# facebookresearch/actionmesh

Measured on AMD Instinct MI355X. Metric: denoise-steps/sec (16f x 4096tok), higher is better.
Workload: dtype bf16; 1 GPU; headline: Stage-I denoise step, B=2 (CFG) x T=16 frames x N=4096 tokens, width 1024 (8 heads x 128), 21 layers all inflated, S=257 ctx tokens, random-init weights, seeded N(0,1) latents/context resident in HBM; parallelism=single GPU

## Files before the change

actionmesh_amd/csrc/am_gemm.hip:

```cpp
#include <stdlib.h>
#include <string.h>

#include "am_common.h"

namespace {

constexpr int BM = 128, BN = 128, BK = 64;
constexpr int LDS_ROW = BK + 8;
constexpr int TILE_ELEMS = BM * LDS_ROW;
constexpr int CS_LD = BN + 4;
constexpr int SMEM_MAIN = 2 * 2 * TILE_ELEMS * (int)sizeof(bf16_t);
constexpr int SMEM_EPI = BM * CS_LD * (int)sizeof(float);
constexpr int SMEM_BYTES = SMEM_MAIN > SMEM_EPI ? SMEM_MAIN : SMEM_EPI;
constexpr int GROUP_M = 8;
constexpr int B2 = 256;

__device__ inline int64_t map_row(int r, int G, int gs, int off) {
  if (G <= 0) return r;
  int g = r / G;
  return (int64_t)g * gs + off + (r - g * G);
}

__global__ __launch_bounds__(256, 2) void gemm_bf16_kernel(am_gemm_args p, int tiles_m, int tiles_n, int m_base) {
  extern __shared__ __attribute__((aligned(16))) unsigned char smem[];
// ... 231 lines not shown
  if (p.residual) {
    const u32x2_t rv = *reinterpret_cast<const u32x2_t*>(p.residual + (int64_t)gmr * p.ldc + gn);
    v[0] += bflo(rv[0]); v[1] += bfhi(rv[0]); v[2] += bflo(rv[1]); v[3] += bfhi(rv[1]);
  }
  *reinterpret_cast<u32x2_t*>(p.C + (int64_t)gmr * p.ldc + gn) = u32x2_t{pack_bf2(v[0], v[1]), pack_bf2(v[2], v[3])};
}

#ifndef AM_GEMM_NT
#define AM_GEMM_NT 1
#endif
struct ResidualPrefetch {
  u32x4_t rv[16];
  bool on;
};
__device__ __forceinline__ bool residual_prefetchable(const am_gemm_args& p, int tid, int m0, int n0) {
  return p.residual != nullptr && p.c_G <= 0 && m0 + B2 <= p.M && n0 + (tid & 31) * 8 < p.N && !(p.act & 0x1800);
}
__device__ __forceinline__ void residual_prefetch(const am_gemm_args& p, int tid, int m0, int n0, ResidualPrefetch& r) {
  r.on = residual_prefetchable(p, tid, m0, n0);
  if (r.on) {
    const int k16 = tid & 31, r16 = tid >> 5;
    const uint32_t lane_off = ((uint32_t)r16 * (uint32_t)p.ldc + (uint32_t)(n0 + k16 * 8)) * 2u;
    const int64_t step = (int64_t)16 * p.ldc;
    const bf16_t* rrow = p.residual + (int64_t)m0 * p.ldc;
#pragma unroll
    for (int pass = 0; pass < 16; ++pass) {
      const u32x4_t* q = reinterpret_cast<const u32x4_t*>(reinterpret_cast<const unsigned char*>(rrow + pass * step) + lane_off);
      r.rv[pass] = AM_GEMM_NT ? __builtin_nontemporal_load(q) : *q;
    }
  }
}

__device__ __forceinline__ void emit_row_part(const u32x4_t& sv, float* part_row, bool writer) {
  float x[8];
#pragma unroll
  for (int e = 0; e < 4; ++e) { x[2 * e] = bflo(sv[e]); x[2 * e + 1] = bfhi(sv[e]); }
  float mean, m2;
  row_part8(x, mean, m2);
#define AM_CHAN_STEP(CTRL, ROWMASK, HALF_N)                                                                                  \
  {                                                                                                                          \
    const float om = __builtin_bit_cast(float, __builtin_amdgcn_update_dpp(__builtin_bit_cast(int, mean), __builtin_bit_cast(int, mean), CTRL, ROWMASK, 0xf, false)); \
    const float oq = __builtin_bit_cast(float, __builtin_amdgcn_update_dpp(__builtin_bit_cast(int, m2), __builtin_bit_cast(int, m2), CTRL, ROWMASK, 0xf, false));     \
    row_part_merge_equal(mean, m2, om, oq, HALF_N);                                                                          \
  }
  AM_CHAN_STEP(0xB1, 0xf, 4.f)
  AM_CHAN_STEP(0x4E, 0xf, 8.f)
  AM_CHAN_STEP(0x141, 0xf, 16.f)
  AM_CHAN_STEP(0x140, 0xf, 32.f)
  AM_CHAN_STEP(0x142, 0xa, 64.f)
#undef AM_CHAN_STEP
  if (writer) *reinterpret_cast<f32x2_t*>(part_row) = f32x2_t{mean, m2};
}

__device__ __forceinline__ void store_staged_tile(const am_gemm_args& p, const unsigned char* stage, int tid, int m0, int n0,
                                                  const ResidualPrefetch* pre = nullptr) {
  {
    const int k16 = tid & 31, r16 = tid >> 5;
    const int gn = n0 + k16 * 8;
    if (gn < p.N) {
      const unsigned char* su = stage + r16 * 512 + ((k16 ^ (r16 >> 1)) << 4);
      const bool odd = r16 & 1;
      auto fetch = [&](int pass) __attribute__((always_inline)) {
        u32x4_t sv = *reinterpret_cast<const u32x4_t*>(su + pass * 8192);
        if (odd) sv = u32x4_t{sv[2], sv[3], sv[0], sv[1]};
        return sv;
      };
      auto add_res = [&](u32x4_t sv, const bf16_t* rp) __attribute__((always_inline)) {
        const u32x4_t rv = *reinterpret_cast<const u32x4_t*>(rp);
#pragma unroll
        for (int e = 0; e < 4; ++e) sv[e] = pack_bf2(bflo(sv[e]) + bflo(rv[e]), bfhi(sv[e]) + bfhi(rv[e]));
// ... 42 lines not shown
        }
      } else {
#pragma unroll 2
        for (int pass = 0; pass < 16; ++pass) {
          const int gmr = m0 + pass * 16 + r16;
          if (gmr < p.M) {
            u32x4_t sv = fetch(pass);
            const int64_t pr = map_row(gmr, p.c_G, p.c_gs, p.c_off);
            if (p.residual) sv = add_res(sv, p.residual + pr * p.ldc + gn);
            *reinterpret_cast<u32x4_t*>(p.C + pr * p.ldc + gn) = sv;
          }
        }
      }
    }
  }
}

__device__ __forceinline__ void store_staged_tile_headpost(const am_gemm_args& p, const am_headpost_args& hp, const unsigned char* stage,
                                                           int tid, int m0, int n0) {
  const int k16 = tid & 31, r16 = tid >> 5;
  const int half = k16 >> 4, sub = k16 & 15;
  const bool abl_noqk = (p.act & 0x800) != 0, abl_nov = (p.act & 0x1000) != 0;
  if (!abl_noqk) {
    const int pi = (n0 >> 7) + half;
    const int head = pi / hp.nparts, part = pi - head * hp.nparts;
    const int kind = (n0 + half * 128 < p.N) ? hp.kinds[part] : 3;
    if (kind == 0 || kind == 1) {
      const float* wt = kind == 0 ? hp.w_q : hp.w_k;
      float wv[8];
#pragma unroll
// ... 310 lines not shown
__device__ __forceinline__ bool gelu_table_has(float x) {
  const uint32_t b = pack_bf2(x, 0.f) & 0x7fffu;
  return b - GT_LO < GT_SPAN;
}

constexpr int HT_BYTES = 128 * BK * 2;
constexpr int PBUF_BYTES = 4 * HT_BYTES;
constexpr int FOLD_OFF = 2 * PBUF_BYTES;
constexpr int SMEM2PP_BYTES = FOLD_OFF + 4096;
constexpr int GT_OFF = SMEM2PP_BYTES;
constexpr int SMEM2PP_GELU_BYTES = GT_OFF + GT_BYTES;

#define PP_BARRIER() do { __builtin_amdgcn_sched_barrier(0); asm volatile("s_barrier" ::: "memory"); __builtin_amdgcn_sched_barrier(0); } while (0)
#define PP_LGKM0() asm volatile("s_waitcnt lgkmcnt(0)" ::: "memory")

template <bool HP>
__global__ __launch_bounds__(512, 2) void gemm256pp_bf16_kernel(am_gemm_args p, int tiles_m, int tiles_n, int m_base, am_headpost_args hp,
                                                                 const uint16_t* gelu_tab) {
  extern __shared__ __attribute__((aligned(16))) unsigned char smem[];

  const int nb = tiles_m * tiles_n;
  const int bid = blockIdx.x;
  {
    const int units = (p.act >> 13) & 7;
    if (units && units < 7 && bid < 256) {
      const unsigned long long t0 = wall_clock64();
      const unsigned long long wait = (unsigned long long)(bid & 7) * units * 150ull;
      while (wall_clock64() - t0 < wait) __builtin_amdgcn_s_sleep(4);
    }
  }
  int lid;
  {
    const int xcd = bid & 7, idx = bid >> 3;
    const int q = nb >> 3, r = nb & 7;
    lid = (xcd < r ? xcd * (q + 1) : r * (q + 1) + (xcd - r) * q) + idx;
  }
  int tm, tn;
  {
    const int group_sz = GROUP_M * tiles_n;
    const int g = lid / group_sz;
    const int first_m = g * GROUP_M;
    const int gm = min(GROUP_M, tiles_m - first_m);
    const int in_g = lid - g * group_sz;
    tm = first_m + in_g % gm;
    tn = in_g / gm;
  }
  const int m0 = m_base + tm * B2, n0 = tn * B2;

  const int tid = threadIdx.x;
  const int lane = tid & 63;
  const int wave = __builtin_amdgcn_readfirstlane(tid >> 6);
  const int wm = wave >> 2, wn = wave & 3;

  const int l15 = lane & 15, l4 = lane >> 4;
  f32x4_t acc[8][4];
  {
    f32x4_t bv[4];
#pragma unroll
    for (int ni = 0; ni < 4; ++ni) {
      bv[ni] = f32x4_t{0.f, 0.f, 0.f, 0.f};
      if (p.bias && !p.ln_stats) bv[ni] = *reinterpret_cast<const f32x4_t*>(p.bias + min(n0 + wn * 64 + ni * 16 + l4 * 4, p.N - 4));
    }
#pragma unroll
    for (int ni = 0; ni < 4; ++ni) asm volatile("" : "+v"(bv[ni]));
#pragma unroll
    for (int ni = 0; ni < 4; ++ni)
#pragma unroll
      for (int mi = 0; mi < 8; ++mi) acc[mi][ni] = bv[ni];
  }
  __builtin_amdgcn_sched_barrier(0);
  if (p.ln_stats) {
    {
      const int dw = wave * 64 + lane;
      const int row = min(m0 + (dw >> 1), p.M - 1);
      __builtin_amdgcn_global_load_lds((gbl_ptr_t)(p.ln_stats + 2 * (int64_t)row + (dw & 1)), (lds_ptr_t)(smem + FOLD_OFF + wave * 256), 4, 0, 0);
    }
    {
      const int idx = (wave & 3) * 64 + lane;
      const int n = min(n0 + idx, p.N - 1);
      const float* src = wave < 4 ? p.ln_colsum + n : (p.bias ? p.bias + n : p.ln_colsum + n);
      __builtin_amdgcn_global_load_lds((gbl_ptr_t)src, (lds_ptr_t)(smem + FOLD_OFF + 2048 + wave * 256), 4, 0, 0);
    }
  }

  if (gelu_tab != nullptr) {
#pragma unroll
    for (int i = 0; i < GT_BYTES / 4 / 512; ++i)
      __builtin_amdgcn_global_load_lds((gbl_ptr_t)(reinterpret_cast<const uint32_t*>(gelu_tab) + i * 512 + wave * 64 + lane),
                                       (lds_ptr_t)(smem + GT_OFF + (i * 512 + wave * 64) * 4), 4, 0, 0);
  }

  uint32_t offA1[4], offA2[4], offW[4];
#pragma unroll
  for (int i = 0; i < 4; ++i) {
    const int half = i >> 1, pc = i & 1;
    const int r = pc * 64 + wave * 8 + (lane >> 3);
    const int c = (lane & 7) ^ ((r >> 1) & 7);
    const int ar = min(m0 + half * 128 + r, p.M - 1);
    const int64_t pr = map_row(ar, p.a_G, p.a_gs, p.a_off);
    offA1[i] = (uint32_t)(pr * (p.lda1 >> 3) + c);
    offA2[i] = (uint32_t)(pr * (p.lda2 >> 3) + c);
    const int wr = min(n0 + half * 128 + r, p.N - 1);
    offW[i] = (uint32_t)((int64_t)wr * (p.ldw >> 3) + c);
  }
  auto stage_a = [&](int half, int kt, int buf_off) __attribute__((always_inline)) {
    const int k0 = kt * BK;
    const bool first = k0 < p.K1;
    const unsigned char* base = reinterpret_cast<const unsigned char*>(first ? p.A1 + k0 : p.A2 + (k0 - p.K1));
#pragma unroll
    for (int pc = 0; pc < 2; ++pc) {
      const uint32_t off = first ? offA1[half * 2 + pc] : offA2[half * 2 + pc];
      __builtin_amdgcn_global_load_lds((gbl_ptr_t)(base + ((uint64_t)off << 4)),
                                       (lds_ptr_t)(smem + buf_off + half * HT_BYTES + (pc * 512 + wave * 64) * 16), 16, 0, 0);
    }
  };
  auto stage_w = [&](int half, int kt, int buf_off) __attribute__((always_inline)) {
    const unsigned char* base = reinterpret_cast<const unsigned char*>(p.W + kt * BK);
#pragma unroll
    for (int pc = 0; pc < 2; ++pc)
      __builtin_amdgcn_global_load_lds((gbl_ptr_t)(base + ((uint64_t)offW[half * 2 + pc] << 4)),
                                       (lds_ptr_t)(smem + buf_off + (2 + half) * HT_BYTES + (pc * 512 + wave * 64) * 16), 16, 0, 0);
  };


  const int fo0 = l15 * 128 + (((0 + l4) ^ (l15 >> 1)) << 4);
  const int fo1 = l15 * 128 + (((4 + l4) ^ (l15 >> 1)) << 4);
  const int a_base = wm * HT_BYTES;
  const int w_base = (2 + (wn >> 1)) * HT_BYTES + (wn & 1) * 64 * 128;

  bf16x8_t af[4][2], wf[4][2];
  auto read_a = [&](int cur, int mh) __attribute__((always_inline)) {
#pragma unroll
    for (int i = 0; i < 4; ++i) {
      const unsigned char* q = smem + cur + a_base + (mh * 4 + i) * 2048;
      af[i][0] = *reinterpret_cast<const bf16x8_t*>(q + fo0);
      af[i][1] = *reinterpret_cast<const bf16x8_t*>(q + fo1);
    }
  };
  auto read_w = [&](int cur, int nh) __attribute__((always_inline)) {
#pragma unroll
    for (int j = 0; j < 2; ++j) {
      const unsigned char* q = smem + cur + w_base + (nh * 2 + j) * 2048;
      wf[nh * 2 + j][0] = *reinterpret_cast<const bf16x8_t*>(q + fo0);
      wf[nh * 2 + j][1] = *reinterpret_cast<const bf16x8_t*>(q + fo1);
    }
  };
#define PP_QUADRANT(MH, NH)                                                                                       \
  do {                                                                                                            \
    __builtin_amdgcn_s_setprio(1);                                                                                \
    _Pragma("unroll") for (int ks = 0; ks < 2; ++ks)                                                              \
      _Pragma("unroll") for (int i = 0; i < 4; ++i)                                                               \
        _Pragma("unroll") for (int j = 0; j < 2; ++j)                                                             \
          acc[(MH) * 4 + i][(NH) * 2 + j] = AM_MFMA_16x16x32(                                                     \
              wf[(NH) * 2 + j][ks], af[i][ks], acc[(MH) * 4 + i][(NH) * 2 + j]);                                  \
    __builtin_amdgcn_s_setprio(0);                                                                                \
  } while (0)

  const int nk = p.K / BK;
  stage_a(0, 0, 0); stage_a(1, 0, 0); stage_w(0, 0, 0); stage_w(1, 0, 0);
  {
    const int t1 = min(1, nk - 1);
    stage_w(0, t1, PBUF_BYTES); stage_w(1, t1, PBUF_BYTES);
  }
  asm volatile("s_waitcnt vmcnt(4)" ::: "memory");
  PP_BARRIER();
  if (wm == 1) PP_BARRIER();

  for (int t = 0; t < nk; ++t) {
    const int cur = (t & 1) * PBUF_BYTES, nxt = PBUF_BYTES - cur;
    const int ta = min(t + 1, nk - 1), tb = min(t + 2, nk - 1);
    read_a(cur, 0); read_w(cur, 0);
    stage_a(0, ta, nxt);
    PP_LGKM0(); PP_BARRIER();
    PP_QUADRANT(0, 0);
    PP_BARRIER();
    read_w(cur, 1);
    stage_a(1, ta, nxt);
    PP_LGKM0(); PP_BARRIER();
    PP_QUADRANT(0, 1);
    PP_BARRIER();
    read_a(cur, 1);
    stage_w(0, tb, cur);
    PP_LGKM0(); PP_BARRIER();
    PP_QUADRANT(1, 1);
    PP_BARRIER();
    stage_w(1, tb, cur);
    asm volatile("s_waitcnt vmcnt(4)" ::: "memory");
    PP_BARRIER();
    PP_QUADRANT(1, 0);
    PP_BARRIER();
  }
  if (wm == 0) PP_BARRIER();
  asm volatile("s_waitcnt vmcnt(0)" ::: "memory");
  PP_BARRIER();

  ResidualPrefetch pre;
  pre.on = false;
  if constexpr (!HP) residual_prefetch(p, tid, m0, n0, pre);
  if (p.ln_stats) {
    f32x4_t cs[4], dv[4];
    const float* fold = reinterpret_cast<const float*>(smem + FOLD_OFF);
#pragma unroll
    for (int ni = 0; ni < 4; ++ni) {
      const int nl = wn * 64 + ni * 16 + l4 * 4;
      cs[ni] = *reinterpret_cast<const f32x4_t*>(fold + 512 + nl);
      dv[ni] = p.bias ? *reinterpret_cast<const f32x4_t*>(fold + 768 + nl) : f32x4_t{0.f, 0.f, 0.f, 0.f};
    }
#pragma unroll
    for (int mi = 0; mi < 8; ++mi) {
      const f32x2_t st = *reinterpret_cast<const f32x2_t*>(fold + 2 * (wm * 128 + mi * 16 + l15));
      const float nm = -st[0] * st[1];
#pragma unroll
      for (int ni = 0; ni < 4; ++ni)
#pragma unroll
        for (int e = 0; e < 4; ++e) acc[mi][ni][e] = fmaf(acc[mi][ni][e], st[1], fmaf(nm, cs[ni][e], dv[ni][e]));
    }
  }
  unsigned char* stage = smem;
  uint32_t gelu_bad = 0;
  auto stage_pass = [&](auto&& convert) __attribute__((always_inline)) {
#pragma unroll
    for (int mi = 0; mi < 8; ++mi)
#pragma unroll
      for (int ni = 0; ni < 4; ++ni) {
        const int ml = wm * 128 + mi * 16 + l15;
        const int nl = wn * 64 + ni * 16 + l4 * 4;
        const u32x2_t w = convert(acc[mi][ni]);
        const int u = (nl >> 2) ^ (ml & 15);
        *reinterpret_cast<u32x2_t*>(stage + ml * 512 + u * 8) = w;
      }
  };
  if ((p.act & 0xff) == 1 && gelu_tab != nullptr) {
    stage_pass([&](const f32x4_t& a) __attribute__((always_inline)) {
      return u32x2_t{gelu_table_pair(pack_bf2(a[0], a[1]), smem + GT_OFF, gelu_bad), gelu_table_pair(pack_bf2(a[2], a[3]), smem + GT_OFF, gelu_bad)};
    });
  } else if ((p.act & 0xff) == 1) {
    stage_pass([&](const f32x4_t& a) __attribute__((always_inline)) {
      float v[4];
#pragma unroll
      for (int e = 0; e < 4; ++e) v[e] = gelu_erf(rbf(a[e]));
      return u32x2_t{pack_bf2(v[0], v[1]), pack_bf2(v[2], v[3])};
    });
  } else {
    stage_pass([&](const f32x4_t& a) __attribute__((always_inline)) { return u32x2_t{pack_bf2(a[0], a[1]), pack_bf2(a[2], a[3])}; });
  }
  if (gelu_bad) {
#pragma unroll
    for (int mi = 0; mi < 8; ++mi)
#pragma unroll
      for (int ni = 0; ni < 4; ++ni) {
        const int ml = wm * 128 + mi * 16 + l15;
        const int nl = wn * 64 + ni * 16 + l4 * 4;
        bool any = false;
#pragma unroll
        for (int e = 0; e < 4; ++e) any |= !gelu_table_has(acc[mi][ni][e]);
        if (any) {
          uint16_t* q = reinterpret_cast<uint16_t*>(stage + ml * 512 + ((nl >> 2) ^ (ml & 15)) * 8);
#pragma unroll
          for (int e = 0; e < 4; ++e)
            if (!gelu_table_has(acc[mi][ni][e])) q[e] = (uint16_t)(pack_bf2(gelu_erf(rbf(acc[mi][ni][e])), 0.f) & 0xffffu);
        }
      }
  }
  __syncthreads();
  if constexpr (HP) store_staged_tile_headpost(p, hp, stage, tid, m0, n0);
  else store_staged_tile(p, stage, tid, m0, n0, &pre);
}
#undef PP_QUADRANT

}

static int gemm_skew_units(int rounds) {
  static int enabled[64];
  int dev = 0;
  if (hipGetDevice(&dev) != hipSuccess || dev < 0 || dev >= 64) return 0;
  if (enabled[dev] == 0) {
    hipDeviceProp_t pr;
    bool on = hipGetDeviceProperties(&pr, dev) == hipSuccess && pr.multiProcessorCount == 256 && strncmp(pr.gcnArchName, "gfx950", 6) == 0;
    const char* e = getenv("ACTIONMESH_AMD_GEMM_SKEW");
    if (e && e[0] == '0') on = false;
    enabled[dev] = on ? 1 : 2;
  }
  if (enabled[dev] != 1) return 0;
  return rounds >= 24 ? 4 : rounds >= 16 ? 3 : rounds >= 12 ? 2 : rounds >= 4 ? 1 : 0;
}

static const uint16_t* gelu_table(hipStream_t st) {
#ifdef AM_F16
  return nullptr;
#else
  static uint16_t* tab[64];
  static int state[64];
  static std::mutex mu;
  int dev = 0, cur = 0;
  if (hipGetDevice(&cur) != hipSuccess) return nullptr;
  dev = cur;
  if (st != nullptr && hipStreamGetDevice(st, &dev) != hipSuccess) { (void)hipGetLastError(); dev = cur; }
  if (dev < 0 || dev >= 64) return nullptr;
  std::lock_guard<std::mutex> lk(mu);
// ... 62 lines not shown
    AM_HIP(hipFuncSetAttribute(reinterpret_cast<const void*>(gemm_bf16_kernel),
                               hipFuncAttributeMaxDynamicSharedMemorySize, SMEM_BYTES));
    AM_HIP(hipFuncSetAttribute(reinterpret_cast<const void*>(gemm256_bf16_kernel),
                               hipFuncAttributeMaxDynamicSharedMemorySize, SMEM2_BYTES));
    AM_HIP(hipFuncSetAttribute(reinterpret_cast<const void*>(gemm256pp_bf16_kernel<false>),
                               hipFuncAttributeMaxDynamicSharedMemorySize, SMEM2PP_GELU_BYTES));
    AM_HIP(hipFuncSetAttribute(reinterpret_cast<const void*>(gemm256pp_bf16_kernel<true>),
                               hipFuncAttributeMaxDynamicSharedMemorySize, SMEM2PP_BYTES));
  });
  am_gemm_args args = *a;
  const bool force_small = (args.act & 0x100) != 0;
  const bool legacy = (args.act & 0x200) != 0;
  const bool force_big = (args.act & 0x400) != 0;
  const int abl = args.act & 0xF800;
  const bool no_gelu_table = (args.act & 0x10000) != 0;
  args.act &= 0xff;
  AM_CHECK(args.act == 0 || args.act == 1, "am_gemm_bf16: unknown activation %d", args.act);
  const bool big = !force_small && args.N >= 8 && args.M >= 1 &&
                   (force_big || (args.N >= 256 && args.M >= 1024 && (int64_t)ceil_div(args.M, B2) * ceil_div(args.N, B2) >= 192));
  args.act |= abl;
  float* const ln_part = args.ln_part;
  int64_t part_done = 0;
  args.ln_part = nullptr;
  if (big && (abl >> 13) == 0) {
    const int rounds = (int)(((int64_t)ceil_div(args.M, B2) * ceil_div(args.N, B2)) / 256);
    args.act |= gemm_skew_units(rounds) << 13;
  }
  if (big) {
    const int rem = args.M % B2;
    const int m_main = (rem != 0 && rem <= 128 && args.M > 8 * B2) ? args.M - rem : args.M;
    const int tiles_m = ceil_div(m_main, B2), tiles_n = ceil_div(args.N, B2);
    if (legacy) {
      hipLaunchKernelGGL(gemm256_bf16_kernel, dim3(tiles_m * tiles_n), dim3(512), SMEM2_BYTES,
                         (hipStream_t)stream, args, tiles_m, tiles_n, 0);
    } else {
      am_gemm_args main_args = args;
      if (ln_part && args.N % B2 == 0 && !(args.act & 0x1800)) {
        main_args.ln_part = ln_part;
        part_done = (int64_t)(args.M / B2) * B2;
        if (part_done > m_main) part_done = m_main;
      }
      const uint16_t* gt = ((main_args.act & 0xff) == 1 && !no_gelu_table) ? gelu_table((hipStream_t)stream) : nullptr;
      hipLaunchKernelGGL(gemm256pp_bf16_kernel<false>, dim3(tiles_m * tiles_n), dim3(512), gt ? SMEM2PP_GELU_BYTES : SMEM2PP_BYTES,
                         (hipStream_t)stream, main_args, tiles_m, tiles_n, 0, am_headpost_args{}, gt);
    }
    if (m_main < args.M) launch_tail(args, m_main, (hipStream_t)stream);
  } else {
    const int tiles_m = ceil_div(args.M, BM), tiles_n = ceil_div(args.N, BN);
    hipLaunchKernelGGL(gemm_bf16_kernel, dim3(tiles_m * tiles_n), dim3(256), SMEM_BYTES,
                       (hipStream_t)stream, args, tiles_m, tiles_n, 0);
  }
  AM_HIP(hipGetLastError());
  if (ln_part && part_done < args.M)
    AM_TRY(am_row_part(args.C, args.ldc, part_done, args.M - part_done, args.N, ln_part, stream));
  return AM_OK;
}

int am_head_post_partial(const am_headpost_args* a, int s_min_last, int s_min_other, void* stream);

// ... 22 lines not shown
  AM_TRY(am_head_post_check(hp));
  AM_ONCE_PER_DEVICE({
    AM_HIP(hipFuncSetAttribute(reinterpret_cast<const void*>(gemm256pp_bf16_kernel<true>), hipFuncAttributeMaxDynamicSharedMemorySize, SMEM2PP_BYTES));
    AM_HIP(hipFuncSetAttribute(reinterpret_cast<const void*>(gemm_bf16_kernel), hipFuncAttributeMaxDynamicSharedMemorySize, SMEM_BYTES));
  });
  am_gemm_args args = *g;
  args.act = g->act & 0x1800;
  const int m_main = tail_split ? args.M - rem : args.M;
  const int tiles_m = ceil_div(m_main, B2), tiles_n = ceil_div(args.N, B2);
  {
    const int rounds = (int)(((int64_t)tiles_m * tiles_n) / 256);
    args.act |= gemm_skew_units(rounds) << 13;
  }
  am_gemm_args main_args = args;
  main_args.M = m_main;
  hipLaunchKernelGGL(gemm256pp_bf16_kernel<true>, dim3(tiles_m * tiles_n), dim3(512), SMEM2PP_BYTES, (hipStream_t)stream, main_args, tiles_m,
                     tiles_n, 0, *hp, (const uint16_t*)nullptr);
  if (m_main < args.M) launch_tail(args, m_main, (hipStream_t)stream);
  AM_HIP(hipGetLastError());
  const int s_min_last = hp->seq_len - (args.M - m_main);
  return am_head_post_partial(hp, s_min_last, hp->seq_len, stream);
}
```

actionmesh_amd/ops.py:

```python
from __future__ import annotations

import ctypes as C
from typing import Optional, Sequence, Tuple

import torch

from . import _lib as L

HEAD_DIM = 128


def _stream(device=None) -> int:
    return torch.cuda.current_stream(device).cuda_stream


def _launch(t: torch.Tensor, fn, what: str, *args) -> None:
    with torch.cuda.device(t.device):
        L.check(fn(*args, _stream(t.device)), what, getattr(fn, "_am_lib", None))


H16 = (torch.bfloat16, torch.float16)


def _fn(t_or_dtype, name: str):
# ... 22 lines not shown
    return (x + m - 1) // m * m


def perm16_index(n: int, device=None) -> torch.Tensor:
    k = torch.arange(n, device=device)
    return (k & ~0xC) | ((k & 4) << 1) | ((k & 8) >> 1)


def gemm(a: torch.Tensor, w: torch.Tensor, bias: Optional[torch.Tensor] = None,
         residual: Optional[torch.Tensor] = None, gelu: bool = False,
         a2: Optional[torch.Tensor] = None, out: Optional[torch.Tensor] = None,
         a_map: Tuple[int, int, int] = (0, 0, 0), c_map: Tuple[int, int, int] = (0, 0, 0),
         M: Optional[int] = None, force_small: bool = False, legacy: bool = False,
         force_big: bool = False, ablate: int = 0,
         ln: Optional[Tuple[torch.Tensor, torch.Tensor]] = None, ln_part: Optional[torch.Tensor] = None,
         gelu_table: bool = True) -> torch.Tensor:
    _need(a, H16, "a"); _need(w, a.dtype, "w")
    K1 = a.shape[1]
    K = w.shape[1]
    N = w.shape[0]
    if M is None:
        M = a.shape[0]
    if out is None:
        out = torch.empty((M, N), dtype=a.dtype, device=a.device)
    _need(out, a.dtype, "out")
    g = L.AmGemmArgs()
    g.A1 = a.data_ptr(); g.lda1 = a.stride(0); g.K1 = K1
    g.A2 = _p(a2); g.lda2 = a2.stride(0) if a2 is not None else 0
    if a2 is not None:
        _need(a2, a.dtype, "a2")
        assert K1 + a2.shape[1] == K
    else:
        assert K1 == K
    g.W = w.data_ptr(); g.ldw = w.stride(0)
    g.bias = _p(_need(bias, torch.float32, "bias")) if bias is not None else None
    g.residual = _p(_need(residual, a.dtype, "residual")) if residual is not None else None
    g.C = out.data_ptr(); g.ldc = out.stride(0)
    g.M, g.N, g.K = M, N, K
    g.act = (1 if gelu else 0) | (0x100 if force_small else 0) | (0x200 if legacy else 0) | (0x400 if force_big else 0) | (ablate & 0xF800) \
        | (0 if gelu_table else 0x10000)
    g.a_G, g.a_gs, g.a_off = a_map
    g.c_G, g.c_gs, g.c_off = c_map
    if ln is not None:
        g.ln_stats = _need(ln[0], torch.float32, "ln stats").data_ptr()
        g.ln_colsum = _need(ln[1], torch.float32, "ln colsum").data_ptr()
        assert ln[0].numel() >= 2 * M and ln[1].numel() == N
    if ln_part is not None:
        _need(ln_part, torch.float32, "ln_part")
        assert ln_part.numel() >= 2 * M * ((N + 255) // 256)
        g.ln_part = ln_part.data_ptr()
    _launch(a, _fn(a, "am_gemm_bf16"), "am_gemm_bf16", C.byref(g))
    return out


def row_stats(x: torch.Tensor, eps: float = 1e-5, out: Optional[torch.Tensor] = None) -> torch.Tensor:
# ... 91 lines not shown
        out_k = torch.zeros((nseq, heads, sk_pad, HEAD_DIM), dtype=x.dtype, device=dev)
    if 2 in kinds and out_vt is None:
        out_vt = torch.zeros((nseq, heads, HEAD_DIM, sk_pad), dtype=x.dtype, device=dev)
    a.out_q = _p(out_q); a.sq_pad = out_q.shape[2] if out_q is not None else 0
    a.out_k = _p(out_k); a.out_vt = _p(out_vt)
    a.sk_pad = out_k.shape[2] if out_k is not None else (out_vt.shape[3] if out_vt is not None else 0)
    _launch(x, _fn(x, "am_head_post"), "am_head_post", C.byref(a))
    return out_q, out_k, out_vt


def gemm_head_post(a: torch.Tensor, w: torch.Tensor, heads: int, kinds: Sequence[int], seq_len: int, rows_per_frame: int,
                   w_q: Optional[torch.Tensor] = None, w_k: Optional[torch.Tensor] = None,
                   rope: Optional[Tuple[torch.Tensor, torch.Tensor]] = None, eps: float = 1e-6,
                   out_q: Optional[torch.Tensor] = None, out_k: Optional[torch.Tensor] = None,
                   out_vt: Optional[torch.Tensor] = None, x: Optional[torch.Tensor] = None,
                   bias: Optional[torch.Tensor] = None, ln: Optional[Tuple[torch.Tensor, torch.Tensor]] = None, ablate: int = 0):
    _need(a, H16, "a"); _need(w, a.dtype, "w")
    rows, K = a.shape
    N = w.shape[0]
    assert N == heads * len(kinds) * HEAD_DIM and w.shape[1] == K
    if x is None:
        x = torch.empty((rows, N), dtype=a.dtype, device=a.device)
    nseq = rows // seq_len
    sq_pad, sk_pad = round_up(seq_len, 256), round_up(seq_len, 64)
    dev = a.device
    g = L.AmGemmArgs()
    g.A1 = a.data_ptr(); g.lda1 = a.stride(0); g.K1 = K
    g.W = w.data_ptr(); g.ldw = w.stride(0)
    g.C = x.data_ptr(); g.ldc = x.stride(0)
    g.M, g.N, g.K = rows, N, K
    g.act = ablate & 0x1800
    if bias is not None:
        g.bias = _need(bias, torch.float32, "bias").data_ptr()
    if ln is not None:
        g.ln_stats = _need(ln[0], torch.float32, "ln stats").data_ptr()
        g.ln_colsum = _need(ln[1], torch.float32, "ln colsum").data_ptr()
    h = L.AmHeadPostArgs()
    h.X = x.data_ptr(); h.ldx = x.stride(0)
    h.rows = rows; h.seq_len = seq_len; h.rows_per_frame = rows_per_frame
    h.heads = heads; h.nparts = len(kinds)
    for i, k in enumerate(kinds):
        h.kinds[i] = k
    h.w_q = _p(w_q); h.w_k = _p(w_k); h.eps = eps
    if rope is not None:
        h.rope_cos = _need(rope[0], torch.float32, "rope_cos").data_ptr()
        h.rope_sin = _need(rope[1], torch.float32, "rope_sin").data_ptr()
# ... 397 lines not shown
```

Baseline: 1.627 denoise-steps/s.

## Make 256-tile GEMM persistent with next-tile prologue overlapped into epilogue store

Launches the 256x256 pipelined GEMM with a grid capped at the CU count, so each workgroup loops over several tiles. The next tile's address setup, bias load and first K-stage prefetch are issued inside the staged-store epilogue once the LDS stage has been read. A fast full-tile store path is also added that loads all 16 passes into registers before writing. Kernel args are reread from the kernarg segment to limit register pressure. The aim is to cut launch and tail-wave overhead and hide the prologue behind epilogue stores, at the cost of more register pressure and more complex control flow.

```diff
diff --git a/actionmesh_amd/csrc/am_gemm.hip b/actionmesh_amd/csrc/am_gemm.hip
--- a/actionmesh_amd/csrc/am_gemm.hip
+++ b/actionmesh_amd/csrc/am_gemm.hip
@@ -269,7 +269,7 @@
   bool on;
 };
 __device__ __forceinline__ bool residual_prefetchable(const am_gemm_args& p, int tid, int m0, int n0) {
-  return p.residual != nullptr && p.c_G <= 0 && m0 + B2 <= p.M && n0 + (tid & 31) * 8 < p.N && !(p.act & 0x1800);
+  return p.residual != nullptr && p.c_G <= 0 && m0 + B2 <= p.M && n0 + B2 <= p.N && !(p.act & 0x1800);
 }
 __device__ __forceinline__ void residual_prefetch(const am_gemm_args& p, int tid, int m0, int n0, ResidualPrefetch& r) {
   r.on = residual_prefetchable(p, tid, m0, n0);
@@ -283,6 +283,9 @@
       const u32x4_t* q = reinterpret_cast<const u32x4_t*>(reinterpret_cast<const unsigned char*>(rrow + pass * step) + lane_off);
       r.rv[pass] = AM_GEMM_NT ? __builtin_nontemporal_load(q) : *q;
     }
+  } else {
+#pragma unroll
+    for (int pass = 0; pass < 16; ++pass) r.rv[pass] = u32x4_t{0u, 0u, 0u, 0u};
   }
 }
 
@@ -307,8 +310,53 @@
   if (writer) *reinterpret_cast<f32x2_t*>(part_row) = f32x2_t{mean, m2};
 }
 
+struct NoStagedHook { __device__ __forceinline__ void operator()() const {} };
+template <class Hook = NoStagedHook>
 __device__ __forceinline__ void store_staged_tile(const am_gemm_args& p, const unsigned char* stage, int tid, int m0, int n0,
-                                                  const ResidualPrefetch* pre = nullptr) {
+                                                  const ResidualPrefetch* pre = nullptr, Hook&& staged_read = Hook()) {
+  if (p.c_G <= 0 && m0 + B2 <= p.M && n0 + B2 <= p.N && !(p.act & 0x800)) {
+    const int k16 = tid & 31, r16 = tid >> 5;
+    const int gn = n0 + k16 * 8;
+    const unsigned char* su = stage + r16 * 512 + ((k16 ^ (r16 >> 1)) << 4);
+    const bool odd = r16 & 1;
+    const uint32_t lane_off = ((uint32_t)r16 * (uint32_t)p.ldc + (uint32_t)gn) * 2u;
+    const int64_t step = (int64_t)16 * p.ldc;
+    u32x4_t sv[16];
+    const bool prefetched = pre != nullptr && pre->on;
+#pragma unroll
+    for (int pass = 0; pass < 16; ++pass) {
+      sv[pass] = *reinterpret_cast<const u32x4_t*>(su + pass * 8192);
+      if (odd) sv[pass] = u32x4_t{sv[pass][2], sv[pass][3], sv[pass][0], sv[pass][1]};
+      if (prefetched) {
+#pragma unroll
+        for (int e = 0; e < 4; ++e)
+          sv[pass][e] = pack_bf2(bflo(sv[pass][e]) + bflo(pre->rv[pass][e]), bfhi(sv[pass][e]) + bfhi(pre->rv[pass][e]));
+      }
+    }
+    if (prefetched) {
+    } else if (p.residual && !(p.act & 0x1000)) {
+      const bf16_t* rrow = p.residual + (int64_t)m0 * p.ldc;
+#pragma unroll
+      for (int pass = 0; pass < 16; ++pass) {
+        const u32x4_t rv = *reinterpret_cast<const u32x4_t*>(reinterpret_cast<const unsigned char*>(rrow + pass * step) + lane_off);
+#pragma unroll
+        for (int e = 0; e < 4; ++e) sv[pass][e] = pack_bf2(bflo(sv[pass][e]) + bflo(rv[e]), bfhi(sv[pass][e]) + bfhi(rv[e]));
+      }
+    }
+    staged_read();
+    bf16_t* crow = p.C + (int64_t)m0 * p.ldc;
+    const int nparts = p.N >> 8;
+    float* prow = p.ln_part ? p.ln_part + 2 * ((int64_t)(m0 + r16) * nparts + (n0 >> 8)) : nullptr;
+    const bool pwriter = k16 == 31;
+    const bool nt = AM_GEMM_NT && ((pre != nullptr && pre->on) || !(p.residual && !(p.act & 0x1000)));
+#pragma unroll
+    for (int pass = 0; pass < 16; ++pass) {
+      u32x4_t* q = reinterpret_cast<u32x4_t*>(reinterpret_cast<unsigned char*>(crow + pass * step) + lane_off);
+      if (nt) __builtin_nontemporal_store(sv[pass], q); else *q = sv[pass];
+      if (prow) emit_row_part(sv[pass], prow + (int64_t)pass * 32 * nparts, pwriter);
+    }
+    return;
+  }
   {
     const int k16 = tid & 31, r16 = tid >> 5;
     const int gn = n0 + k16 * 8;
@@ -381,6 +429,7 @@
       }
     }
   }
+  staged_read();
 }
 
 __device__ __forceinline__ void store_staged_tile_headpost(const am_gemm_args& p, const am_headpost_args& hp, const unsigned char* stage,
@@ -721,96 +770,62 @@
 #define PP_BARRIER() do { __builtin_amdgcn_sched_barrier(0); asm volatile("s_barrier" ::: "memory"); __builtin_amdgcn_sched_barrier(0); } while (0)
 #define PP_LGKM0() asm volatile("s_waitcnt lgkmcnt(0)" ::: "memory")
 
+template <bool HP> struct HeadPostParam { am_headpost_args v; };
+template <> struct HeadPostParam<false> { int unused; };
+template <bool HP> struct Gemm256Args {
+  am_gemm_args p;
+  int tiles_m, tiles_n, m_base;
+  HeadPostParam<HP> hpp;
+  const uint16_t* gelu_tab;
+};
+
+#ifdef AM_GEMM_STAMPS
+__device__ unsigned long long* g_gemm_stamps = nullptr;
+#define AM_STAMP(BID, K) do { if (threadIdx.x == 0 && g_gemm_stamps) g_gemm_stamps[(size_t)(BID) * 8 + (K)] = ((K) < 5 ? __builtin_readcyclecounter() : wall_clock64()); } while (0)
+#else
+#define AM_STAMP(BID, K) do { } while (0)
+#endif
+
 template <bool HP>
-__global__ __launch_bounds__(512, 2) void gemm256pp_bf16_kernel(am_gemm_args p, int tiles_m, int tiles_n, int m_base, am_headpost_args hp,
-                                                                 const uint16_t* gelu_tab) {
+__global__ __launch_bounds__(512, 2) void gemm256pp_bf16_kernel(Gemm256Args<HP>) {
   extern __shared__ __attribute__((aligned(16))) unsigned char smem[];
-
-  const int nb = tiles_m * tiles_n;
-  const int bid = blockIdx.x;
+  typedef const __attribute__((address_space(4))) Gemm256Args<HP>* karg_ptr_t;
+  const karg_ptr_t kargs = (karg_ptr_t)__builtin_amdgcn_kernarg_segment_ptr();
+  auto fresh_args = [&]() __attribute__((always_inline)) -> const Gemm256Args<HP>& {
+    karg_ptr_t q = kargs;
+    asm volatile("" : "+s"(q));
+    return *(const Gemm256Args<HP>*)q;
+  };
+  {
+  const am_gemm_args& p = fresh_args().p;
   {
     const int units = (p.act >> 13) & 7;
-    if (units && units < 7 && bid < 256) {
+    if (units && units < 7 && blockIdx.x < 256) {
       const unsigned long long t0 = wall_clock64();
-      const unsigned long long wait = (unsigned long long)(bid & 7) * units * 150ull;
+      const unsigned long long wait = (unsigned long long)(blockIdx.x & 7) * units * 150ull;
       while (wall_clock64() - t0 < wait) __builtin_amdgcn_s_sleep(4);
     }
   }
-  int lid;
-  {
-    const int xcd = bid & 7, idx = bid >> 3;
-    const int q = nb >> 3, r = nb & 7;
-    lid = (xcd < r ? xcd * (q + 1) : r * (q + 1) + (xcd - r) * q) + idx;
-  }
-  int tm, tn;
-  {
-    const int group_sz = GROUP_M * tiles_n;
-    const int g = lid / group_sz;
-    const int first_m = g * GROUP_M;
-    const int gm = min(GROUP_M, tiles_m - first_m);
-    const int in_g = lid - g * group_sz;
-    tm = first_m + in_g % gm;
-    tn = in_g / gm;
-  }
-  const int m0 = m_base + tm * B2, n0 = tn * B2;
-
-  const int tid = threadIdx.x;
-  const int lane = tid & 63;
-  const int wave = __builtin_amdgcn_readfirstlane(tid >> 6);
-  const int wm = wave >> 2, wn = wave & 3;
-
-  const int l15 = lane & 15, l4 = lane >> 4;
-  f32x4_t acc[8][4];
-  {
-    f32x4_t bv[4];
-#pragma unroll
-    for (int ni = 0; ni < 4; ++ni) {
-      bv[ni] = f32x4_t{0.f, 0.f, 0.f, 0.f};
-      if (p.bias && !p.ln_stats) bv[ni] = *reinterpret_cast<const f32x4_t*>(p.bias + min(n0 + wn * 64 + ni * 16 + l4 * 4, p.N - 4));
-    }
-#pragma unroll
-    for (int ni = 0; ni < 4; ++ni) asm volatile("" : "+v"(bv[ni]));
-#pragma unroll
-    for (int ni = 0; ni < 4; ++ni)
-#pragma unroll
-      for (int mi = 0; mi < 8; ++mi) acc[mi][ni] = bv[ni];
-  }
-  __builtin_amdgcn_sched_barrier(0);
-  if (p.ln_stats) {
-    {
-      const int dw = wave * 64 + lane;
-      const int row = min(m0 + (dw >> 1), p.M - 1);
-      __builtin_amdgcn_global_load_lds((gbl_ptr_t)(p.ln_stats + 2 * (int64_t)row + (dw & 1)), (lds_ptr_t)(smem + FOLD_OFF + wave * 256), 4, 0, 0);
-    }
-    {
-      const int idx = (wave & 3) * 64 + lane;
-      const int n = min(n0 + idx, p.N - 1);
-      const float* src = wave < 4 ? p.ln_colsum + n : (p.bias ? p.bias + n : p.ln_colsum + n);
-      __builtin_amdgcn_global_load_lds((gbl_ptr_t)src, (lds_ptr_t)(smem + FOLD_OFF + 2048 + wave * 256), 4, 0, 0);
-    }
-  }
-
-  if (gelu_tab != nullptr) {
+  }
+
+  auto opaque_tid = [&]() __attribute__((always_inline)) {
+    int t = threadIdx.x;
+    asm volatile("" : "+v"(t));
+    return t;
+  };
+
+  if (const uint16_t* gelu_tab = fresh_args().gelu_tab) {
+    const int wave = __builtin_amdgcn_readfirstlane(threadIdx.x >> 6);
 #pragma unroll
     for (int i = 0; i < GT_BYTES / 4 / 512; ++i)
-      __builtin_amdgcn_global_load_lds((gbl_ptr_t)(reinterpret_cast<const uint32_t*>(gelu_tab) + i * 512 + wave * 64 + lane),
+      __builtin_amdgcn_global_load_lds((gbl_ptr_t)(reinterpret_cast<const uint32_t*>(gelu_tab) + i * 512 + wave * 64 + (threadIdx.x & 63)),
                                        (lds_ptr_t)(smem + GT_OFF + (i * 512 + wave * 64) * 4), 4, 0, 0);
   }
 
+  int m0 = 0, n0 = 0;
+  f32x4_t bv[4];
   uint32_t offA1[4], offA2[4], offW[4];
-#pragma unroll
-  for (int i = 0; i < 4; ++i) {
-    const int half = i >> 1, pc = i & 1;
-    const int r = pc * 64 + wave * 8 + (lane >> 3);
-    const int c = (lane & 7) ^ ((r >> 1) & 7);
-    const int ar = min(m0 + half * 128 + r, p.M - 1);
-    const int64_t pr = map_row(ar, p.a_G, p.a_gs, p.a_off);
-    offA1[i] = (uint32_t)(pr * (p.lda1 >> 3) + c);
-    offA2[i] = (uint32_t)(pr * (p.lda2 >> 3) + c);
-    const int wr = min(n0 + half * 128 + r, p.N - 1);
-    offW[i] = (uint32_t)((int64_t)wr * (p.ldw >> 3) + c);
-  }
-  auto stage_a = [&](int half, int kt, int buf_off) __attribute__((always_inline)) {
+  auto stage_a = [&](const am_gemm_args& p, int wave, int half, int kt, int buf_off) __attribute__((always_inline)) {
     const int k0 = kt * BK;
     const bool first = k0 < p.K1;
     const unsigned char* base = reinterpret_cast<const unsigned char*>(first ? p.A1 + k0 : p.A2 + (k0 - p.K1));
@@ -821,37 +836,73 @@
                                        (lds_ptr_t)(smem + buf_off + half * HT_BYTES + (pc * 512 + wave * 64) * 16), 16, 0, 0);
     }
   };
-  auto stage_w = [&](int half, int kt, int buf_off) __attribute__((always_inline)) {
+  auto stage_w = [&](const am_gemm_args& p, int wave, int half, int kt, int buf_off) __attribute__((always_inline)) {
     const unsigned char* base = reinterpret_cast<const unsigned char*>(p.W + kt * BK);
 #pragma unroll
     for (int pc = 0; pc < 2; ++pc)
       __builtin_amdgcn_global_load_lds((gbl_ptr_t)(base + ((uint64_t)offW[half * 2 + pc] << 4)),
                                        (lds_ptr_t)(smem + buf_off + (2 + half) * HT_BYTES + (pc * 512 + wave * 64) * 16), 16, 0, 0);
   };
-
-
-  const int fo0 = l15 * 128 + (((0 + l4) ^ (l15 >> 1)) << 4);
-  const int fo1 = l15 * 128 + (((4 + l4) ^ (l15 >> 1)) << 4);
-  const int a_base = wm * HT_BYTES;
-  const int w_base = (2 + (wn >> 1)) * HT_BYTES + (wn & 1) * 64 * 128;
-
-  bf16x8_t af[4][2], wf[4][2];
-  auto read_a = [&](int cur, int mh) __attribute__((always_inline)) {
+  auto open_tile = [&](int bid) __attribute__((always_inline)) {
+    const int tid_o = opaque_tid();
+    const int lane_o = tid_o & 63, wave = __builtin_amdgcn_readfirstlane(tid_o >> 6), wn = wave & 3;
+    const int l4 = lane_o >> 4;
+    const Gemm256Args<HP>& ka = fresh_args();
+    const am_gemm_args& p = ka.p;
+    const int tiles_m = ka.tiles_m, tiles_n = ka.tiles_n, nb = tiles_m * tiles_n, nk = p.K / BK;
+    int lid;
+    {
+      const int xcd = bid & 7, idx = bid >> 3;
+      const int q = nb >> 3, r = nb & 7;
+      lid = (xcd < r ? xcd * (q + 1) : r * (q + 1) + (xcd - r) * q) + idx;
+    }
+    int tm, tn;
+    {
+      const int group_sz = GROUP_M * tiles_n;
+      const int g = lid / group_sz;
+      const int first_m = g * GROUP_M;
+      const int gm = min(GROUP_M, tiles_m - first_m);
+      const int in_g = lid - g * group_sz;
+      tm = first_m + in_g % gm;
+      tn = in_g / gm;
+    }
+    m0 = ka.m_base + tm * B2;
+    n0 = tn * B2;
+#pragma unroll
+    for (int ni = 0; ni < 4; ++ni) {
+      bv[ni] = f32x4_t{0.f, 0.f, 0.f, 0.f};
+      if (p.bias && !p.ln_stats) bv[ni] = *reinterpret_cast<const f32x4_t*>(p.bias + min(n0 + wn * 64 + ni * 16 + l4 * 4, p.N - 4));
+    }
+    if (p.ln_stats) {
+      {
+        const int dw = wave * 64 + lane_o;
+        const int row = min(m0 + (dw >> 1), p.M - 1);
+        __builtin_amdgcn_global_load_lds((gbl_ptr_t)(p.ln_stats + 2 * (int64_t)row + (dw & 1)), (lds_ptr_t)(smem + FOLD_OFF + wave * 256), 4, 0, 0);
+      }
+      {
+        const int idx = (wave & 3) * 64 + lane_o;
+        const int n = min(n0 + idx, p.N - 1);
+        const float* src = wave < 4 ? p.ln_colsum + n : (p.bias ? p.bias + n : p.ln_colsum + n);
+        __builtin_amdgcn_global_load_lds((gbl_ptr_t)src, (lds_ptr_t)(smem + FOLD_OFF + 2048 + wave * 256), 4, 0, 0);
+      }
+    }
 #pragma unroll
     for (int i = 0; i < 4; ++i) {
-      const unsigned char* q = smem + cur + a_base + (mh * 4 + i) * 2048;
-      af[i][0] = *reinterpret_cast<const bf16x8_t*>(q + fo0);
-      af[i][1] = *reinterpret_cast<const bf16x8_t*>(q + fo1);
-    }
+      const int half = i >> 1, pc = i & 1;
+      const int r = pc * 64 + wave * 8 + (lane_o >> 3);
+      const int c = (lane_o & 7) ^ ((r >> 1) & 7);
+      const int ar = min(m0 + half * 128 + r, p.M - 1);
+      const int64_t pr = map_row(ar, p.a_G, p.a_gs, p.a_off);
+      offA1[i] = (uint32_t)(pr * (p.lda1 >> 3) + c);
+      offA2[i] = (uint32_t)(pr * (p.lda2 >> 3) + c);
+      const int wr = min(n0 + half * 128 + r, p.N - 1);
+      offW[i] = (uint32_t)((int64_t)wr * (p.ldw >> 3) + c);
+    }
+    stage_a(p, wave, 0, 0, 0); stage_a(p, wave, 1, 0, 0); stage_w(p, wave, 0, 0, 0); stage_w(p, wave, 1, 0, 0);
+    const int t1 = min(1, nk - 1);
+    stage_w(p, wave, 0, t1, PBUF_BYTES); stage_w(p, wave, 1, t1, PBUF_BYTES);
   };
-  auto read_w = [&](int cur, int nh) __attribute__((always_inline)) {
-#pragma unroll
-    for (int j = 0; j < 2; ++j) {
-      const unsigned char* q = smem + cur + w_base + (nh * 2 + j) * 2048;
-      wf[nh * 2 + j][0] = *reinterpret_cast<const bf16x8_t*>(q + fo0);
-      wf[nh * 2 + j][1] = *reinterpret_cast<const bf16x8_t*>(q + fo1);
-    }
-  };
+
 #define PP_QUADRANT(MH, NH)                                                                                       \
   do {                                                                                                            \
     __builtin_amdgcn_s_setprio(1);                                                                                \
@@ -863,115 +914,181 @@
     __builtin_amdgcn_s_setprio(0);                                                                                \
   } while (0)
 
-  const int nk = p.K / BK;
-  stage_a(0, 0, 0); stage_a(1, 0, 0); stage_w(0, 0, 0); stage_w(1, 0, 0);
-  {
-    const int t1 = min(1, nk - 1);
-    stage_w(0, t1, PBUF_BYTES); stage_w(1, t1, PBUF_BYTES);
-  }
-  asm volatile("s_waitcnt vmcnt(4)" ::: "memory");
-  PP_BARRIER();
-  if (wm == 1) PP_BARRIER();
-
-  for (int t = 0; t < nk; ++t) {
-    const int cur = (t & 1) * PBUF_BYTES, nxt = PBUF_BYTES - cur;
-    const int ta = min(t + 1, nk - 1), tb = min(t + 2, nk - 1);
-    read_a(cur, 0); read_w(cur, 0);
-    stage_a(0, ta, nxt);
-    PP_LGKM0(); PP_BARRIER();
-    PP_QUADRANT(0, 0);
+  AM_STAMP(blockIdx.x, 0); AM_STAMP(blockIdx.x, 5);
+  open_tile(blockIdx.x);
+  for (int bid = blockIdx.x;;) {
+    const int tm0 = m0, tn0 = n0;
+    asm volatile("s_waitcnt vmcnt(0)" ::: "memory");
     PP_BARRIER();
-    read_w(cur, 1);
-    stage_a(1, ta, nxt);
-    PP_LGKM0(); PP_BARRIER();
-    PP_QUADRANT(0, 1);
+    f32x4_t acc[8][4];
+#pragma unroll
+    for (int ni = 0; ni < 4; ++ni)
+#pragma unroll
+      for (int mi = 0; mi < 8; ++mi) acc[mi][ni] = bv[ni];
+    const int tid_m = opaque_tid();
+    const int lane_m = tid_m & 63, wave = __builtin_amdgcn_readfirstlane(tid_m >> 6);
+    const int wm = wave >> 2, wn = wave & 3;
+    const int f15 = lane_m & 15, f4 = lane_m >> 4;
+    const int fo0 = f15 * 128 + (((0 + f4) ^ (f15 >> 1)) << 4);
+    const int fo1 = f15 * 128 + (((4 + f4) ^ (f15 >> 1)) << 4);
+    const int a_base = wm * HT_BYTES;
+    const int w_base = (2 + (wn >> 1)) * HT_BYTES + (wn & 1) * 64 * 128;
+
+    bf16x8_t af[4][2], wf[4][2];
+    auto read_a = [&](int cur, int mh) __attribute__((always_inline)) {
+  #pragma unroll
+      for (int i = 0; i < 4; ++i) {
+        const unsigned char* q = smem + cur + a_base + (mh * 4 + i) * 2048;
+        af[i][0] = *reinterpret_cast<const bf16x8_t*>(q + fo0);
+        af[i][1] = *reinterpret_cast<const bf16x8_t*>(q + fo1);
+      }
+    };
+    auto read_w = [&](int cur, int nh) __attribute__((always_inline)) {
+  #pragma unroll
+      for (int j = 0; j < 2; ++j) {
+        const unsigned char* q = smem + cur + w_base + (nh * 2 + j) * 2048;
+        wf[nh * 2 + j][0] = *reinterpret_cast<const bf16x8_t*>(q + fo0);
+        wf[nh * 2 + j][1] = *reinterpret_cast<const bf16x8_t*>(q + fo1);
+      }
+    };
+    if (wm == 1) PP_BARRIER();
+    AM_STAMP(bid, 1);
+
+    {
+    am_gemm_args p;
+    {
+      const am_gemm_args& q = fresh_args().p;
+      p.A1 = q.A1; p.A2 = q.A2; p.W = q.W; p.K1 = q.K1; p.K = q.K;
+      asm volatile("" : "+s"(p.A1), "+s"(p.A2), "+s"(p.W), "+s"(p.K1), "+s"(p.K));
+    }
+    const int nk = p.K / BK;
+    for (int t = 0; t < nk; ++t) {
+      const int cur = (t & 1) * PBUF_BYTES, nxt = PBUF_BYTES - cur;
+      const int ta = min(t + 1, nk - 1), tb = min(t + 2, nk - 1);
+      read_a(cur, 0); read_w(cur, 0);
+      stage_a(p, wave, 0, ta, nxt);
+      PP_LGKM0(); PP_BARRIER();
+      PP_QUADRANT(0, 0);
+      PP_BARRIER();
+      read_w(cur, 1);
+      stage_a(p, wave, 1, ta, nxt);
+      PP_LGKM0(); PP_BARRIER();
+      PP_QUADRANT(0, 1);
+      PP_BARRIER();
+      read_a(cur, 1);
+      stage_w(p, wave, 0, tb, cur);
+      PP_LGKM0(); PP_BARRIER();
+      PP_QUADRANT(1, 1);
+      PP_BARRIER();
+      stage_w(p, wave, 1, tb, cur);
+      asm volatile("s_waitcnt vmcnt(4)" ::: "memory");
+      PP_BARRIER();
+      PP_QUADRANT(1, 0);
+      PP_BARRIER();
+    }
+    }
+    if (wm == 0) PP_BARRIER();
+    asm volatile("s_waitcnt vmcnt(0)" ::: "memory");
     PP_BARRIER();
-    read_a(cur, 1);
-    stage_w(0, tb, cur);
-    PP_LGKM0(); PP_BARRIER();
-    PP_QUADRANT(1, 1);
-    PP_BARRIER();
-    stage_w(1, tb, cur);
-    asm volatile("s_waitcnt vmcnt(4)" ::: "memory");
-    PP_BARRIER();
-    PP_QUADRANT(1, 0);
-    PP_BARRIER();
-  }
-  if (wm == 0) PP_BARRIER();
-  asm volatile("s_waitcnt vmcnt(0)" ::: "memory");
-  PP_BARRIER();
-
-  ResidualPrefetch pre;
-  pre.on = false;
-  if constexpr (!HP) residual_prefetch(p, tid, m0, n0, pre);
-  if (p.ln_stats) {
-    f32x4_t cs[4], dv[4];
-    const float* fold = reinterpret_cast<const float*>(smem + FOLD_OFF);
-#pragma unroll
-    for (int ni = 0; ni < 4; ++ni) {
-      const int nl = wn * 64 + ni * 16 + l4 * 4;
-      cs[ni] = *reinterpret_cast<const f32x4_t*>(fold + 512 + nl);
-      dv[ni] = p.bias ? *reinterpret_cast<const f32x4_t*>(fold + 768 + nl) : f32x4_t{0.f, 0.f, 0.f, 0.f};
-    }
-#pragma unroll
-    for (int mi = 0; mi < 8; ++mi) {
-      const f32x2_t st = *reinterpret_cast<const f32x2_t*>(fold + 2 * (wm * 128 + mi * 16 + l15));
-      const float nm = -st[0] * st[1];
-#pragma unroll
-      for (int ni = 0; ni < 4; ++ni)
-#pragma unroll
-        for (int e = 0; e < 4; ++e) acc[mi][ni][e] = fmaf(acc[mi][ni][e], st[1], fmaf(nm, cs[ni][e], dv[ni][e]));
-    }
-  }
-  unsigned char* stage = smem;
-  uint32_t gelu_bad = 0;
-  auto stage_pass = [&](auto&& convert) __attribute__((always_inline)) {
-#pragma unroll
-    for (int mi = 0; mi < 8; ++mi)
+    AM_STAMP(bid, 2);
+
+    const Gemm256Args<HP>& ka = fresh_args();
+    const am_gemm_args& p = ka.p;
+    const uint16_t* const gelu_tab = ka.gelu_tab;
+    const int tid_e = opaque_tid();
+    const int l15 = tid_e & 15, l4 = (tid_e >> 4) & 3;
+    if (p.ln_stats) {
+      f32x4_t cs[4], dv[4];
+      const float* fold = reinterpret_cast<const float*>(smem + FOLD_OFF);
 #pragma unroll
       for (int ni = 0; ni < 4; ++ni) {
-        const int ml = wm * 128 + mi * 16 + l15;
         const int nl = wn * 64 + ni * 16 + l4 * 4;
-        const u32x2_t w = convert(acc[mi][ni]);
-        const int u = (nl >> 2) ^ (ml & 15);
-        *reinterpret_cast<u32x2_t*>(stage + ml * 512 + u * 8) = w;
-      }
-  };
-  if ((p.act & 0xff) == 1 && gelu_tab != nullptr) {
-    stage_pass([&](const f32x4_t& a) __attribute__((always_inline)) {
-      return u32x2_t{gelu_table_pair(pack_bf2(a[0], a[1]), smem + GT_OFF, gelu_bad), gelu_table_pair(pack_bf2(a[2], a[3]), smem + GT_OFF, gelu_bad)};
-    });
-  } else if ((p.act & 0xff) == 1) {
-    stage_pass([&](const f32x4_t& a) __attribute__((always_inline)) {
-      float v[4];
-#pragma unroll
-      for (int e = 0; e < 4; ++e) v[e] = gelu_erf(rbf(a[e]));
-      return u32x2_t{pack_bf2(v[0], v[1]), pack_bf2(v[2], v[3])};
-    });
-  } else {
-    stage_pass([&](const f32x4_t& a) __attribute__((always_inline)) { return u32x2_t{pack_bf2(a[0], a[1]), pack_bf2(a[2], a[3])}; });
-  }
-  if (gelu_bad) {
-#pragma unroll
-    for (int mi = 0; mi < 8; ++mi)
-#pragma unroll
-      for (int ni = 0; ni < 4; ++ni) {
-        const int ml = wm * 128 + mi * 16 + l15;
-        const int nl = wn * 64 + ni * 16 + l4 * 4;
-        bool any = false;
-#pragma unroll
-        for (int e = 0; e < 4; ++e) any |= !gelu_table_has(acc[mi][ni][e]);
-        if (any) {
-          uint16_t* q = reinterpret_cast<uint16_t*>(stage + ml * 512 + ((nl >> 2) ^ (ml & 15)) * 8);
-#pragma unroll
-          for (int e = 0; e < 4; ++e)
-            if (!gelu_table_has(acc[mi][ni][e])) q[e] = (uint16_t)(pack_bf2(gelu_erf(rbf(acc[mi][ni][e])), 0.f) & 0xffffu);
+        cs[ni] = *reinterpret_cast<const f32x4_t*>(fold + 512 + nl);
+        dv[ni] = p.bias ? *reinterpret_cast<const f32x4_t*>(fold + 768 + nl) : f32x4_t{0.f, 0.f, 0.f, 0.f};
+      }
+#pragma unroll
+      for (int mi = 0; mi < 8; ++mi) {
+        const f32x2_t st = *reinterpret_cast<const f32x2_t*>(fold + 2 * (wm * 128 + mi * 16 + l15));
+        const float nm = -st[0] * st[1];
+#pragma unroll
+        for (int ni = 0; ni < 4; ++ni)
+#pragma unroll
+          for (int e = 0; e < 4; ++e) acc[mi][ni][e] = fmaf(acc[mi][ni][e], st[1], fmaf(nm, cs[ni][e], dv[ni][e]));
+      }
+    }
+    ResidualPrefetch pre;
+    pre.on = false;
+    if constexpr (!HP) residual_prefetch(p, tid_e, tm0, tn0, pre);
+    unsigned char* stage = smem;
+    uint32_t gelu_bad = 0;
+    auto stage_pass = [&](auto&& convert) __attribute__((always_inline)) {
+#pragma unroll
+      for (int mi = 0; mi < 8; ++mi)
+#pragma unroll
+        for (int ni = 0; ni < 4; ++ni) {
+          const int ml = wm * 128 + mi * 16 + l15;
+          const int nl = wn * 64 + ni * 16 + l4 * 4;
+          const u32x2_t w = convert(acc[mi][ni]);
+          const int u = (nl >> 2) ^ (ml & 15);
+          *reinterpret_cast<u32x2_t*>(stage + ml * 512 + u * 8) = w;
         }
-      }
-  }
-  __syncthreads();
-  if constexpr (HP) store_staged_tile_headpost(p, hp, stage, tid, m0, n0);
-  else store_staged_tile(p, stage, tid, m0, n0, &pre);
+    };
+    if ((p.act & 0xff) == 1 && gelu_tab != nullptr) {
+      stage_pass([&](const f32x4_t& a) __attribute__((always_inline)) {
+        return u32x2_t{gelu_table_pair(pack_bf2(a[0], a[1]), smem + GT_OFF, gelu_bad), gelu_table_pair(pack_bf2(a[2], a[3]), smem + GT_OFF, gelu_bad)};
+      });
+    } else if ((p.act & 0xff) == 1) {
+      stage_pass([&](const f32x4_t& a) __attribute__((always_inline)) {
+        float v[4];
+#pragma unroll
+        for (int e = 0; e < 4; ++e) v[e] = gelu_erf(rbf(a[e]));
+        return u32x2_t{pack_bf2(v[0], v[1]), pack_bf2(v[2], v[3])};
+      });
+    } else {
+      stage_pass([&](const f32x4_t& a) __attribute__((always_inline)) { return u32x2_t{pack_bf2(a[0], a[1]), pack_bf2(a[2], a[3])}; });
+    }
+    if (gelu_bad) {
+#pragma unroll
+      for (int mi = 0; mi < 8; ++mi)
+#pragma unroll
+        for (int ni = 0; ni < 4; ++ni) {
+          const int ml = wm * 128 + mi * 16 + l15;
+          const int nl = wn * 64 + ni * 16 + l4 * 4;
+          bool any = false;
+#pragma unroll
+          for (int e = 0; e < 4; ++e) any |= !gelu_table_has(acc[mi][ni][e]);
+          if (any) {
+            uint16_t* q = reinterpret_cast<uint16_t*>(stage + ml * 512 + ((nl >> 2) ^ (ml & 15)) * 8);
+#pragma unroll
+            for (int e = 0; e < 4; ++e)
+              if (!gelu_table_has(acc[mi][ni][e])) q[e] = (uint16_t)(pack_bf2(gelu_erf(rbf(acc[mi][ni][e])), 0.f) & 0xffffu);
+          }
+        }
+    }
+    __syncthreads();
+    AM_STAMP(bid, 3);
+    const int nbid = bid + (int)gridDim.x;
+    const bool more = nbid < ka.tiles_m * ka.tiles_n;
+    auto staged_read = [&]() __attribute__((always_inline)) {
+      if (more) {
+        PP_LGKM0(); PP_BARRIER();
+        open_tile(nbid);
+      } else {
+#pragma unroll
+        for (int i = 0; i < 4; ++i) { bv[i] = f32x4_t{0.f, 0.f, 0.f, 0.f}; offA1[i] = offA2[i] = offW[i] = 0u; }
+      }
+    };
+    if constexpr (HP) {
+      store_staged_tile_headpost(p, ka.hpp.v, stage, tid_e, tm0, tn0);
+      staged_read();
+    } else {
+      store_staged_tile(p, stage, tid_e, tm0, tn0, &pre, staged_read);
+    }
+    AM_STAMP(bid, 4); AM_STAMP(bid, 6);
+    if (!more) break;
+    bid = nbid;
+    AM_STAMP(bid, 0); AM_STAMP(bid, 5);
+  }
 }
 #undef PP_QUADRANT
 
@@ -990,6 +1107,27 @@
   }
   if (enabled[dev] != 1) return 0;
   return rounds >= 24 ? 4 : rounds >= 16 ? 3 : rounds >= 12 ? 2 : rounds >= 4 ? 1 : 0;
+}
+
+#ifdef AM_GEMM_STAMPS
+extern "C" int am_gemm_stamps_bind(unsigned long long* buf) {
+  AM_HIP(hipMemcpyToSymbol(HIP_SYMBOL(g_gemm_stamps), &buf, sizeof(buf)));
+  return AM_OK;
+}
+#endif
+
+static int gemm_grid(int tiles, bool one_tile_per_workgroup) {
+  static int cus[64];
+  int dev = 0;
+  if (one_tile_per_workgroup || hipGetDevice(&dev) != hipSuccess || dev < 0 || dev >= 64) return tiles;
+  if (cus[dev] == 0) {
+    hipDeviceProp_t pr;
+    int n = hipGetDeviceProperties(&pr, dev) == hipSuccess && pr.multiProcessorCount > 0 ? pr.multiProcessorCount : -1;
+    const char* e = getenv("ACTIONMESH_AMD_GEMM_PERSISTENT");
+    if (e && e[0] == '0') n = -1;
+    cus[dev] = n;
+  }
+  return cus[dev] > 0 && cus[dev] < tiles ? cus[dev] : tiles;
 }
 
 static const uint16_t* gelu_table(hipStream_t st) {
@@ -1082,6 +1220,7 @@
   const bool force_big = (args.act & 0x400) != 0;
   const int abl = args.act & 0xF800;
   const bool no_gelu_table = (args.act & 0x10000) != 0;
+  const bool one_tile = (args.act & 0x20000) != 0;
   args.act &= 0xff;
   AM_CHECK(args.act == 0 || args.act == 1, "am_gemm_bf16: unknown activation %d", args.act);
   const bool big = !force_small && args.N >= 8 && args.M >= 1 &&
@@ -1109,8 +1248,8 @@
         if (part_done > m_main) part_done = m_main;
       }
       const uint16_t* gt = ((main_args.act & 0xff) == 1 && !no_gelu_table) ? gelu_table((hipStream_t)stream) : nullptr;
-      hipLaunchKernelGGL(gemm256pp_bf16_kernel<false>, dim3(tiles_m * tiles_n), dim3(512), gt ? SMEM2PP_GELU_BYTES : SMEM2PP_BYTES,
-                         (hipStream_t)stream, main_args, tiles_m, tiles_n, 0, am_headpost_args{}, gt);
+      hipLaunchKernelGGL(gemm256pp_bf16_kernel<false>, dim3(gemm_grid(tiles_m * tiles_n, one_tile)), dim3(512), gt ? SMEM2PP_GELU_BYTES : SMEM2PP_BYTES,
+                         (hipStream_t)stream, Gemm256Args<false>{main_args, tiles_m, tiles_n, 0, {0}, gt});
     }
     if (m_main < args.M) launch_tail(args, m_main, (hipStream_t)stream);
   } else {
@@ -1163,8 +1302,8 @@
   }
   am_gemm_args main_args = args;
   main_args.M = m_main;
-  hipLaunchKernelGGL(gemm256pp_bf16_kernel<true>, dim3(tiles_m * tiles_n), dim3(512), SMEM2PP_BYTES, (hipStream_t)stream, main_args, tiles_m,
-                     tiles_n, 0, *hp, (const uint16_t*)nullptr);
+  hipLaunchKernelGGL(gemm256pp_bf16_kernel<true>, dim3(gemm_grid(tiles_m * tiles_n, (g->act & 0x20000) != 0)), dim3(512), SMEM2PP_BYTES,
+                     (hipStream_t)stream, Gemm256Args<true>{main_args, tiles_m, tiles_n, 0, {*hp}, nullptr});
   if (m_main < args.M) launch_tail(args, m_main, (hipStream_t)stream);
   AM_HIP(hipGetLastError());
   const int s_min_last = hp->seq_len - (args.M - m_main);
diff --git a/actionmesh_amd/ops.py b/actionmesh_amd/ops.py
--- a/actionmesh_amd/ops.py
+++ b/actionmesh_amd/ops.py
@@ -60,7 +60,7 @@
          M: Optional[int] = None, force_small: bool = False, legacy: bool = False,
          force_big: bool = False, ablate: int = 0,
          ln: Optional[Tuple[torch.Tensor, torch.Tensor]] = None, ln_part: Optional[torch.Tensor] = None,
-         gelu_table: bool = True) -> torch.Tensor:
+         gelu_table: bool = True, one_tile: bool = False) -> torch.Tensor:
     _need(a, H16, "a"); _need(w, a.dtype, "w")
     K1 = a.shape[1]
     K = w.shape[1]
@@ -84,7 +84,7 @@
     g.C = out.data_ptr(); g.ldc = out.stride(0)
     g.M, g.N, g.K = M, N, K
     g.act = (1 if gelu else 0) | (0x100 if force_small else 0) | (0x200 if legacy else 0) | (0x400 if force_big else 0) | (ablate & 0xF800) \
-        | (0 if gelu_table else 0x10000)
+        | (0 if gelu_table else 0x10000) | (0x20000 if one_tile else 0)
     g.a_G, g.a_gs, g.a_off = a_map
     g.c_G, g.c_gs, g.c_off = c_map
     if ln is not None:
@@ -206,7 +206,8 @@
                    rope: Optional[Tuple[torch.Tensor, torch.Tensor]] = None, eps: float = 1e-6,
                    out_q: Optional[torch.Tensor] = None, out_k: Optional[torch.Tensor] = None,
                    out_vt: Optional[torch.Tensor] = None, x: Optional[torch.Tensor] = None,
-                   bias: Optional[torch.Tensor] = None, ln: Optional[Tuple[torch.Tensor, torch.Tensor]] = None, ablate: int = 0):
+                   bias: Optional[torch.Tensor] = None, ln: Optional[Tuple[torch.Tensor, torch.Tensor]] = None, ablate: int = 0,
+                   one_tile: bool = False):
     _need(a, H16, "a"); _need(w, a.dtype, "w")
     rows, K = a.shape
     N = w.shape[0]
@@ -222,6 +223,8 @@
     g.C = x.data_ptr(); g.ldc = x.stride(0)
     g.M, g.N, g.K = rows, N, K
     g.act = ablate & 0x1800
+    if one_tile:
+        g.act |= 0x20000
     if bias is not None:
         g.bias = _need(bias, torch.float32, "bias").data_ptr()
     if ln is not None:
```

Result: no change. 1.624 denoise-steps/s (-0.2%).
